# paninski-lab/lightning-pose

Hardware: AMD Instinct MI355X
Metric: training frames/sec (whole node), ResNet-50 384x384 17-kp semi-sup (higher is better)
Workload: dtype bf16; 1 GPU; C2/C3: ResNet-50 SemiSupervisedHeatmapTracker 384x384, K=17, 64 labeled + 128 unlabeled frames per GPU, heatmap_mse + temporal + pca_singleview + unimodal_mse, Adam (backbone lr=0 as at step 0), bf16-mixed; global_batch=192, parallelism=dp1, sync_batchnorm=False, decode_prune=plain kernels (chosen from the maps)

## Files before the change

include/lp_hip.h:

```cpp
#ifndef LP_HIP_H
#define LP_HIP_H

#include <stddef.h>
#include <stdint.h>

#ifdef __cplusplus
extern "C" {
#endif

typedef void* lp_stream_t;

int lp_config_reload_env(void);

enum {
    LP_OK = 0,
    LP_ERR_ARGUMENT = -1,
    LP_ERR_UNSUPPORTED = -2,
};

enum { LP_TF_NONE = 0, LP_TF_SINGLE = 1, LP_TF_PER_FRAME = 2, LP_TF_PER_VIEW = 3 };

#define LP_HIP_ABI_VERSION 142
int lp_version(void);
const char* lp_strerror(int code);


typedef struct lp_decode_tables {
    const int* row_base;
    const float* row_taps;
    const int* col_start;
    const float* col_taps;
    const int* colT_start;
    const float* colT_taps;
    int ty, tx, tc;
} lp_decode_tables;

typedef struct lp_frame_map {
    const float* transforms;
    int tf_mode;
    const float* bbox;
    int bbox_stride;
    int kp_per_view;
    float model_h, model_w;
} lp_frame_map;

// ... 49 lines not shown

int lp_temporal_fwd_bwd(const float* kp, const float* conf, int S, int K, const float* eps_per_kp, float prob_threshold,
                        float* loss, float* grad_unit, lp_stream_t stream);

int lp_pca_fwd_bwd(const float* kp, int S, int K, const int* index, int rows, int points, const float* mean,
                   const float* kept_eigenvectors, int ncomp, float epsilon, float* loss, float* grad_unit, lp_stream_t stream);

int lp_rmse_fwd(const float* kp_targ, const float* kp_pred, int n_points, float* loss, lp_stream_t stream);
int lp_loss_combine(const float* const* x, const float* w, const float* a, int n, float* weighted, float* total, lp_stream_t stream);
int lp_loss_combine_bwd(const float* w, const float* a, int n, const float* g_weighted, const float* g_total, float* gx, lp_stream_t stream);

typedef struct lp_conv_geom {
    int B, Hi, Wi, Ci;
    int Ho, Wo, Co;
    int R, S, stride, pad;
} lp_conv_geom;

#define LP_CONV_KERNEL_IGEMM 0
#define LP_CONV_KERNEL_PIPE 1
#define LP_CONV_KERNEL_WGRAD 2
#define LP_CONV_KERNEL_WGRAD_PIPE 3
#define LP_CONV_KERNEL_PIPE_HALO 4
#define LP_CONV_KERNEL_STEM_WGRAD_NB 8
#define LP_CONV_KERNEL_RES2D 5
int lp_conv_last_kernel(void);

int lp_conv_fwd(const void* x, const void* w, const lp_conv_geom* geom, const float* bias, void* out_bf16, float* out_f32, int ldo,
                int n_store, lp_stream_t stream);
int lp_conv_dgrad(const void* dy, const void* wd, const lp_conv_geom* geom, const float* bias, const void* addend,
                  const void* relu_mask, void* dx_bf16, float* dx_f32, int ldo, int n_store, int skip_empty_classes,
                  lp_stream_t stream);
typedef struct lp_gemm_batch {
    int nb, nh;
    long long a_b, a_h, b_b, b_h, c_b, c_h;
} lp_gemm_batch;
int lp_gemm_nt(const void* a, int lda, const void* b, int ldb, void* c_bf16, float* c_f32, int ldc, int M, int N, int K, int n_store,
               const float* bias, const lp_gemm_batch* batch, lp_stream_t stream);
int lp_gemm_tn(const void* x, int ldx, const void* y, int ldy, void* out_bf16, int ldo, int M, int J, int N, const lp_gemm_batch* batch,
               lp_stream_t stream);
int lp_attn_fwd(const void* qkv_bf16, int ld_qkv, int k_off, int v_off, int B, int nh, int T, float scale, void* p_bf16, int ldp,
                void* out_bf16, int ldo, lp_stream_t stream);
int lp_attn_bwd_kv(const void* qkv_bf16, int ld_qkv, int v_off, const void* d_out_bf16, int ld_do, const void* p_bf16, int ldp, const float* d_rows,
                   int B, int nh, int T, float scale, void* ds_bf16, void* dqkv_bf16, int ld_dqkv, int dk_off, int dv_off, lp_stream_t stream);
int lp_attn_rowdot(const void* a_bf16, const void* b_bf16, int rows, int nh, int ld, float* out, lp_stream_t stream);
int lp_attn_dscores(const void* d_out, int ld_do, const void* v, int ldv, const void* p_bf16, const float* d_rows, int d_row_stride,
                    long long d_b, long long d_h, float scale, void* ds_bf16, int ldc, int M, int N, int K, const lp_gemm_batch* batch,
// ... 174 lines not shown
```

lightning-pose_amd/_lib.py:

```python

from __future__ import annotations

import ctypes as C
import os

_HERE = os.path.dirname(os.path.abspath(__file__))
LIB_PATH = os.environ.get("LP_HIP_LIB") or os.path.join(_HERE, "liblp_hip.so")


class LpHipUnavailable(RuntimeError):
    """liblp_hip.so could not be loaded, or an op was given a non-ROCm tensor.  There is no fallback path."""


class LpHipError(RuntimeError):
    pass


class DecodeTables(C.Structure):
    _fields_ = [("row_base", C.c_void_p), ("row_taps", C.c_void_p), ("col_start", C.c_void_p),
                ("col_taps", C.c_void_p), ("colT_start", C.c_void_p), ("colT_taps", C.c_void_p),
                ("ty", C.c_int), ("tx", C.c_int), ("tc", C.c_int)]


class FrameMap(C.Structure):
# ... 6 lines not shown


class BnFuse(C.Structure):
    _fields_ = [("z", C.c_void_p), ("mean", C.c_void_p), ("invstd", C.c_void_p), ("gamma", C.c_void_p), ("beta", C.c_void_p),
                ("mask_from_z", C.c_int), ("relu_bits", C.c_void_p), ("sums", C.c_void_p), ("seg_images", C.c_int), ("addend_half", C.c_int)]


class FrameNorm(C.Structure):
    _fields_ = [("mean", C.c_float * 3), ("std", C.c_float * 3)]


class FrameAugment(C.Structure):
    _fields_ = [("has_matrix", C.c_int), ("matrix", C.c_float * 6), ("brightness", C.c_float), ("contrast", C.c_float),
                ("contrast_center", C.c_float), ("shot_factor", C.c_float), ("seed", C.c_ulonglong)]


class GemmBatch(C.Structure):
    _fields_ = [("nb", C.c_int), ("nh", C.c_int)] + [(n, C.c_longlong) for n in ("a_b", "a_h", "b_b", "b_h", "c_b", "c_h")]


HM_MSE, HM_KL, HM_JS = 0, 1, 2
CONV_KERNEL_IGEMM, CONV_KERNEL_PIPE, CONV_KERNEL_WGRAD, CONV_KERNEL_WGRAD_PIPE, CONV_KERNEL_PIPE_HALO, CONV_KERNEL_RES2D = 0, 1, 2, 3, 4, 5
CONV_KERNEL_STEM_WGRAD_NB = 8
BORDER_RENORM, BORDER_CLAMP = 0, 1
TF_NONE, TF_SINGLE, TF_PER_FRAME, TF_PER_VIEW = 0, 1, 2, 3

ABI_VERSION = 142

_P, _I, _F, _L, _Z = C.c_void_p, C.c_int, C.c_float, C.c_long, C.c_size_t

PROTOTYPES = {
    "lp_version": (_I, []),
    "lp_strerror": (C.c_char_p, [_I]),
    "lp_config_reload_env": (_I, []),
    "lp_decode_window": (_I, [_I, _I]),
    "lp_decode_fwd": (_I, [_P, _I, _I, _I, _I, _I, _F, C.POINTER(DecodeTables), C.POINTER(FrameMap), _P, _P, _P, _P, _I, _P]),
    "lp_decode_bwd": (_I, [_P, _I, _I, _I, _I, _I, _F, C.POINTER(DecodeTables), C.POINTER(FrameMap), _P, _P, _P, _P, _I, _I, _P]),
    "lp_frame_map_apply": (_I, [_P, _I, _I, C.POINTER(FrameMap), _I, _P, _P]),
    "lp_heatmap_gen": (_I, [_P, _P, _I, _I, _I, _I, _I, _I, _F, _P, _P]),
    "lp_heatmap_gen_bwd": (_I, [_P, _P, _I, _I, _I, _I, _I, _I, _F, _P, _P, _P]),
    "lp_temporal_heatmap_workspace_bytes": (_Z, [_I, _I]),
    "lp_temporal_heatmap_fwd": (_I, [_I, _P, _P, _I, _I, _I, _I, _P, _F, _P, _P, _P]),
    "lp_temporal_heatmap_bwd": (_I, [_I, _P, _I, _I, _I, _I, _P, _P, _P, _I, _P]),
    "lp_heatmap_confidence": (_I, [_P, _P, _I, _I, _I, _I, _I, _P, _P]),
    "lp_heatmap_mse_workspace_bytes": (_Z, [_I, _I]),
    "lp_heatmap_mse_fwd": (_I, [_P, _P, _I, _I, _I, _I, _P, _P, _P]),
    "lp_heatmap_mse_bwd": (_I, [_P, _P, _I, _I, _I, _I, _P, _P, _P, _I, _P]),
    "lp_heatmap_loss_fwd": (_I, [_I, _P, _P, _I, _I, _I, _I, _P, _P, _P]),
    "lp_heatmap_loss_bwd": (_I, [_I, _P, _P, _I, _I, _I, _I, _P, _P, _P, _I, _P]),
    "lp_unimodal_mse_fwd": (_I, [_P, _P, _P, _I, _I, _I, _I, _I, _I, _F, _F, _P, _P, _P]),
# ... 138 lines not shown
```

lightning-pose_amd/csrc/api.hip:

```cpp
#include "lp_common.h"

#include <stdlib.h>

#include <atomic>

extern "C" int lp_version(void) { return LP_HIP_ABI_VERSION; }

namespace lp {
static int env_int(const char* name, int dflt) {
    const char* e = getenv(name);
    return (e == nullptr || *e == 0) ? dflt : atoi(e);
}
static LpSwitches read_switches() {
    LpSwitches s;
    s.conv_pipe = env_int("LP_CONV_PIPE", 1);
    s.conv_halo = env_int("LP_CONV_HALO", 1);
    s.conv_res2d = env_int("LP_CONV_RES2D", 1);
    s.infer_pipe = env_int("LP_INFER_PIPE", 1);
    s.gemm_pipe = env_int("LP_GEMM_PIPE", 1);
    s.wgrad_pipe = env_int("LP_WGRAD_PIPE", 1);
    s.stem_2d = env_int("LP_STEM_2D", 1);
    s.stem_wgrad_nb = env_int("LP_STEM_WGRAD_NB", 1);
    s.pool_v2 = env_int("LP_POOL_V2", 1);
    s.bn_bwd_wgs_per_cu = env_int("LP_BN_BWD_WGS_PER_CU", 5);
    if (s.bn_bwd_wgs_per_cu < 1 || s.bn_bwd_wgs_per_cu > 5) s.bn_bwd_wgs_per_cu = 5;
    s.conv_max_wgs = env_int("LP_CONV_MAX_WGS", 0);
    return s;
}
static std::atomic<const LpSwitches*> g_switches{new LpSwitches(read_switches())};
const LpSwitches& lp_switches() { return *g_switches.load(std::memory_order_acquire); }
}

extern "C" int lp_config_reload_env(void) {
    lp::g_switches.store(new lp::LpSwitches(lp::read_switches()), std::memory_order_release);
    return LP_OK;
}

extern "C" const char* lp_strerror(int code) {
    if (code == LP_OK) return "ok";
    if (code == LP_ERR_ARGUMENT) return "invalid argument (null pointer or non-positive dimension)";
    if (code == LP_ERR_UNSUPPORTED) return "shape not covered by the instantiated kernels";
    if (code > 0) return hipGetErrorString((hipError_t)code);
    return "unknown lp_hip error";
// ... 2 lines not shown
```

lightning-pose_amd/csrc/conv.hip:

```cpp
#include <stdlib.h>

#include "lp_common.h"

namespace lp {

constexpr int kBM = 128;
constexpr int kBK = 64;
constexpr int kLD = kBK + 8;

struct ConvGeom {
    int B, Hi, Wi, Ci;
    int Ho, Wo, Co;
    int R, S, stride, pad;
};

struct ConvEpilogue {
    unsigned short* out_bf16;
    float* out_f32;
    int ldo;
    int n_store;
    const float* bias;
    const unsigned short* addend;
    const unsigned short* relu_mask;
    const unsigned char* relu_bits;
// ... 509 lines not shown
            if (kt + 1 < KT) load_step(kt + 1);
            mma_kstep<NT>(sA[cur], sB[cur], wm, wn, lane, acc);
            if (kt + 1 < KT) store_step(cur ^ 1);
            __syncthreads();
        }
        vt += gridDim.x;
        const unsigned zd = zdn;
        if (vt >= ntiles) {
            epilogue(m0, n0, zo, zd);
            if (ep.stats_sums != nullptr) stats_flush();
            break;
        }
        setup(vt);
        load_step(0, MODE != kModeDgrad);
        epilogue(m0, n0, zo, zd);
        if (MODE == kModeDgrad) load_b_deferred();
        __syncthreads();
    }
}

}

#include "conv_pipe.h"
#include "conv_res2d.h"

namespace lp {

struct TnExt {
    unsigned short* out;
    int ldx, ldy, ldo;
    int nh;
    unsigned x_zb, x_zh;
    unsigned y_zb, y_zh;
    unsigned o_zb, o_zh;
    float* col_sums;
};

#ifndef LP_WGRAD_DEEP
#define LP_WGRAD_DEEP 1
#endif
constexpr bool kWgradDeep = LP_WGRAD_DEEP != 0;

template <int BN, bool STEM, bool CS = false>
__global__ __launch_bounds__(256) void conv_wgrad_kernel(const unsigned short* __restrict__ X, const unsigned short* __restrict__ DY,
                                                         unsigned x_bytes, unsigned dy_bytes, ConvGeom g, int M, int Kw, int tiles,
                                                         int tiles_n, int m_per_split, FastDiv div_hw, FastDiv div_wo,
// ... 574 lines not shown
    const void *pa = x, *qb = dy;
    unsigned pa_bytes = x_bytes, qb_bytes = dy_bytes;
    if (p.swap) {
        wg = WgradPipeGeom{g.B, g.Ho, g.Wo, g.Ho, g.Wo, g.Co, 1, 1, 1, 0, p.Ka, p.Cb, 1};
        pa = dy, qb = x, pa_bytes = dy_bytes, qb_bytes = x_bytes;
    } else {
        const int plain = g.R == 1 && g.S == 1 && g.stride == 1 && g.pad == 0 && g.Hi == g.Ho && g.Wi == g.Wo;
        wg = WgradPipeGeom{g.B, g.Hi, g.Wi, g.Ho, g.Wo, g.Ci, g.R, g.S, g.stride, g.pad, p.Ka, p.Cb, plain};
    }
    const int tiles = p.tiles_a * p.tiles_b;
    const FastDiv dhw = make_fastdiv(g.Ho * g.Wo), dwo = make_fastdiv(g.Wo);
    g_last_conv_kernel = LP_CONV_KERNEL_WGRAD_PIPE;
    const int sa = p.swap ? Kw : 1, sb = p.swap ? 1 : Kw;
    if (p.bn == 128) {
        hipLaunchKernelGGL((conv_wgrad_pipe_kernel<128>), dim3(tiles * p.split), dim3(512), 0, st, (const unsigned short*)pa,
                           (const unsigned short*)qb, pa_bytes, qb_bytes, wg, M, tiles, p.tiles_b, p.per, dhw, dwo, ws);
        hipLaunchKernelGGL((wgrad_pipe_reduce_kernel<128>), dim3(tiles * 256 * 128 / 64), dim3(256), 0, st, ws, p.split, tiles, p.tiles_b, p.Ka,
                           p.Cb, sa, sb, dw);
    } else {
        hipLaunchKernelGGL((conv_wgrad_pipe_kernel<64>), dim3(tiles * p.split), dim3(512), 0, st, (const unsigned short*)pa,
                           (const unsigned short*)qb, pa_bytes, qb_bytes, wg, M, tiles, p.tiles_b, p.per, dhw, dwo, ws);
        hipLaunchKernelGGL((wgrad_pipe_reduce_kernel<64>), dim3(tiles * 256 * 64 / 64), dim3(256), 0, st, ws, p.split, tiles, p.tiles_b, p.Ka,
                           p.Cb, sa, sb, dw);
    }
}

static bool geom_ok(const lp_conv_geom* c) {
    return c && c->B > 0 && c->Hi > 0 && c->Wi > 0 && c->Ci > 0 && c->Ho > 0 && c->Wo > 0 && c->Co > 0 && c->R > 0 && c->S > 0 &&
           c->stride > 0 && c->pad >= 0;
}

static ConvGeom to_geom(const lp_conv_geom* c) {
    ConvGeom g{c->B, c->Hi, c->Wi, c->Ci, c->Ho, c->Wo, c->Co, c->R, c->S, c->stride, c->pad};
    return g;
}

}

static int conv_fwd_impl(const void* x, const void* w, const lp_conv_geom* geom, const float* bias, void* out_bf16, float* out_f32, int ldo,
                         int n_store, const lp_bn_fuse* bn, lp_stream_t stream) {
    using namespace lp;
    LP_REQUIRE(x && w && geom_ok(geom) && (out_bf16 || out_f32) && ldo > 0);
    ConvGeom g = to_geom(geom);
    if (g.Ci % kBK != 0 || g.R * g.S > 32 || (long long)g.B * g.Hi * g.Wi * g.Ci >= (1LL << 31) ||
        (long long)g.B * g.Ho * g.Wo * ldo >= (1LL << 32))
        return LP_ERR_UNSUPPORTED;
// ... 277 lines not shown
    if (split > ksteps) split = ksteps;
    if (split < 1) split = 1;
    p.per = ((ksteps + split - 1) / split) * lp::kBK;
    p.split = (M + p.per - 1) / p.per;
    p.tj = 2, p.tn = 1, p.wide = false;
    p.ws_floats = (size_t)p.split * 2 * 4 * 2 * 16 * 64;
    return p;
}

extern "C" size_t lp_conv_wgrad_workspace_bytes(const lp_conv_geom* geom, int split_hint) {
    using namespace lp;
    if (!geom_ok(geom)) return 0;
    ConvGeom g = to_geom(geom);
    const bool stem = (g.Ci == 4 && g.R == 7);
    const int Kw = stem ? 256 : g.R * g.S * g.Ci;
    size_t fl = plan_wgrad(g.B * g.Ho * g.Wo, Kw, g.Co, split_hint, kWgradWgs).ws_floats;
    if (stem && stem_wgrad_nb_ok(g)) {
        const size_t nb = plan_stem_wgrad_nb(g.B * g.Ho * g.Wo, split_hint).ws_floats;
        if (nb > fl) fl = nb;
    }
    if (!stem) {
        const WgradPipePlan pp = plan_wgrad_pipe(g, split_hint, true);
        if (pp.ok && pp.ws_floats > fl) fl = pp.ws_floats;
    }
    return fl * sizeof(float);
}

static int conv_wgrad_impl(const void* x, const void* dy, const lp_conv_geom* geom, float* dw, float* dbias, int split_hint, void* workspace,
                           size_t workspace_bytes, lp_stream_t stream) {
    using namespace lp;
    LP_REQUIRE(x && dy && geom_ok(geom) && dw && workspace);
    ConvGeom g = to_geom(geom);
    if (g.Ci % 8 != 0 || g.Co % 8 != 0 || (long long)g.B * g.Hi * g.Wi * g.Ci >= (1LL << 31) ||
        (long long)g.B * g.Ho * g.Wo * g.Co >= (1LL << 31))
        return LP_ERR_UNSUPPORTED;
    const int M = g.B * g.Ho * g.Wo, Kw = g.R * g.S * g.Ci;
    const unsigned x_bytes = (unsigned)(2ull * g.B * g.Hi * g.Wi * g.Ci), dy_bytes = (unsigned)(2ull * M * g.Co);
    const WgradPlan p = plan_wgrad(M, Kw, g.Co, split_hint, kWgradWgs);
    LP_REQUIRE(workspace_bytes >= p.ws_floats * sizeof(float));
    hipStream_t st = (hipStream_t)stream;
    float* ws = (float*)workspace;
    const int wpe = lp_switches().wgrad_pipe;
    if (!dbias && conv_pipe_enabled() && wpe != 0) {
        const WgradPipePlan pp = plan_wgrad_pipe(g, split_hint, wpe == 2);
        if (pp.ok && workspace_bytes >= pp.ws_floats * sizeof(float)) {
            launch_wgrad_pipe(pp, x, dy, g, dw, ws, st);
            return launch_status();
        }
    }
    g_last_conv_kernel = LP_CONV_KERNEL_WGRAD;
    const int tiles = p.tj * p.tn;
    TnExt ext{};
    ext.col_sums = dbias;
    const dim3 grid(tiles * p.split), block(256);
    const FastDiv dhw = make_fastdiv(g.Ho * g.Wo), dwo = make_fastdiv(g.Wo);
    const unsigned short *xs = (const unsigned short*)x, *dys = (const unsigned short*)dy;
#define LP_WGRAD_LAUNCH(BN_, CS_)                                                                                                \
    hipLaunchKernelGGL((conv_wgrad_kernel<BN_, false, CS_>), grid, block, 0, st, xs, dys, x_bytes, dy_bytes, g, M, Kw, tiles, p.tn, \
                       p.per, dhw, dwo, ws, ext)
    if (p.wide) {
        if (dbias) LP_WGRAD_LAUNCH(128, true);
        else LP_WGRAD_LAUNCH(128, false);
        launch_wgrad_reduce<128>(ws, p.split, tiles, p.tn, Kw, g.Co, dw, st);
    } else {
        if (dbias) LP_WGRAD_LAUNCH(64, true);
// ... 117 lines not shown
```

lightning-pose_amd/csrc/conv_pipe.h:

```cpp
#pragma once

#include <type_traits>

namespace lp {

#ifndef LP_HALO_KEY_ROW
#define LP_HALO_KEY_ROW 0
#endif
#ifndef LP_HALO_STAGES
#define LP_HALO_STAGES 3
#endif
#ifndef LP_FWD_CORNER_PAD
#define LP_FWD_CORNER_PAD 0
#endif
#ifndef LP_PIPE_SPREAD
#define LP_PIPE_SPREAD 1
#endif
constexpr bool kSpread = LP_PIPE_SPREAD != 0;
constexpr int kPM = 256;
constexpr int kPRowB = 128;

#if defined(__HIP_DEVICE_COMPILE__)
#define LP_WAIT_VM(n) asm volatile("s_waitcnt vmcnt(" #n ")" ::: "memory")
#define LP_RAW_BARRIER()                   \
    do {                                   \
        asm volatile("" ::: "memory");     \
        __builtin_amdgcn_s_barrier();      \
        asm volatile("" ::: "memory");     \
    } while (0)
#define LP_WAIT_LGKM_TOUCH3(n, a, b, c) asm volatile("s_waitcnt lgkmcnt(" #n ")" : "+v"(a), "+v"(b), "+v"(c)::"memory")
#define LP_WAIT_LGKM_TOUCH4(n, a, b, c, d) asm volatile("s_waitcnt lgkmcnt(" #n ")" : "+v"(a), "+v"(b), "+v"(c), "+v"(d)::"memory")
#else
#define LP_WAIT_VM(n) ((void)0)
#define LP_RAW_BARRIER() __syncthreads()
#define LP_WAIT_LGKM_TOUCH3(n, a, b, c) ((void)0)
#define LP_WAIT_LGKM_TOUCH4(n, a, b, c, d) ((void)0)
#endif

__device__ __forceinline__ void store8(unsigned short* p, u16x8 v) { *reinterpret_cast<u16x8*>(p) = v; }
// ... 669 lines not shown
    const int bchunk = (BN == 128) ? ((lane & 15) ^ ((brow & 3) << 2)) : ((lane & 7) ^ (((brow >> 1) & 1) << 2));
    const unsigned boff = (unsigned)(b0 + bchunk * 8) * 2u;
    const int hw = g.Ho * g.Wo;

    unsigned is_a[4], is_b[NLB];
    unsigned char* is_dst = smem;
    const bool same = !g.plain && g.stride == 1 && g.Hi == g.Ho && g.Wi == g.Wo && hw >= kBK;
    const int qb64 = kBK / hw, qh64 = (kBK - qb64 * hw) / g.Wo, qw64 = kBK - qb64 * hw - qh64 * g.Wo;
    const int lo_h = max(0, g.pad - tr), span_h = min(g.Ho, g.Hi + g.pad - tr) - lo_h;
    const int lo_w = max(0, g.pad - ts), span_w = min(g.Wo, g.Wi + g.pad - ts) - lo_w;
    const unsigned tap_off = (unsigned)(((tr - g.pad) * g.Wi + (ts - g.pad)) * g.Ca + tcn) * 2u;
    int rho[4], rwo[4];
    if (same) {
#pragma unroll
        for (int p = 0; p < 4; ++p) {
            const int m = m_begin + p * 16 + arow;
            const int mm = m < M ? m : 0;
            const int rem = mm - fdiv(mm, div_hw) * hw;
            rho[p] = fdiv(rem, div_wo);
            rwo[p] = rem - rho[p] * g.Wo;
        }
    }
    auto prep_step = [&](int st, int kt) {
        const int mk = m_begin + kt * kBK;
#pragma unroll
        for (int p = 0; p < 4; ++p) {
            const int m = mk + p * 16 + arow;
            unsigned off;
            bool ok = ja_ok && m < m_end && kt < KT;
            if (g.plain) {
                off = (unsigned)(m * g.Ca + tcn) * 2u;
            } else if (same) {
                ok = ok && (unsigned)(rho[p] - lo_h) < (unsigned)span_h && (unsigned)(rwo[p] - lo_w) < (unsigned)span_w;
                off = (unsigned)m * (unsigned)(g.Ca * 2) + tap_off;
                rwo[p] += qw64;
                const int c = rwo[p] >= g.Wo ? 1 : 0;
                rwo[p] -= c ? g.Wo : 0;
                rho[p] += qh64 + c;
                rho[p] -= rho[p] >= g.Ho ? g.Ho : 0;
            } else {
                const int mm = ok ? m : 0;
                const int b = fdiv(mm, div_hw), rem = mm - b * hw;
                const int ho = fdiv(rem, div_wo), wo = rem - ho * g.Wo;
                const int hi = ho * g.stride - g.pad + tr, wi = wo * g.stride - g.pad + ts;
                ok = ok && hi >= 0 && hi < g.Hi && wi >= 0 && wi < g.Wi;
                off = (unsigned)(((b * g.Hi + hi) * g.Wi + wi) * g.Ca + tcn) * 2u;
            }
// ... 27 lines not shown
        const int e0 = wn * (NT * 32) + nt * 32 + fcol;
        fob[nt] = (unsigned)(kStageA + frow * kRowB + (((e0 >> 3) ^ swb) << 4) + (e0 & 7) * 2);
    }
    f32x16 acc[2][NT];
#pragma unroll
    for (int mt = 0; mt < 2; ++mt)
#pragma unroll
        for (int nt = 0; nt < NT; ++nt)
#pragma unroll
            for (int e = 0; e < 16; ++e) acc[mt][nt][e] = 0.f;

    auto mma_stage = [&](int st) {
        const unsigned char* sb = smem + st * kStage;
        bf16x8 a[2][2], b[2][NT];
        const unsigned char* pa[2];
        const unsigned char* pb[NT];
#pragma unroll
        for (int mt = 0; mt < 2; ++mt) pa[mt] = sb + foa[mt];
#pragma unroll
        for (int nt = 0; nt < NT; ++nt) pb[nt] = sb + fob[nt];
        auto fetch = [&](auto kk_c, int set) {
            constexpr int kk = decltype(kk_c)::value;
            typedef __attribute__((ext_vector_type(8))) short s16x8_t;
#pragma unroll
            for (int mt = 0; mt < 2; ++mt) {
                const s16x4_t lo = lds_read_tr16_async_off<kk * 16 * kRowA>(pa[mt]), hi = lds_read_tr16_async_off<kk * 16 * kRowA + 4 * kRowA>(pa[mt]);
                const s16x8_t v = {lo[0], lo[1], lo[2], lo[3], hi[0], hi[1], hi[2], hi[3]};
                a[set][mt] = __builtin_bit_cast(bf16x8, v);
            }
#pragma unroll
            for (int nt = 0; nt < NT; ++nt) {
                const s16x4_t lo = lds_read_tr16_async_off<kk * 16 * kRowB>(pb[nt]), hi = lds_read_tr16_async_off<kk * 16 * kRowB + 4 * kRowB>(pb[nt]);
                const s16x8_t v = {lo[0], lo[1], lo[2], lo[3], hi[0], hi[1], hi[2], hi[3]};
                b[set][nt] = __builtin_bit_cast(bf16x8, v);
            }
        };
        auto ready = [&](int set, bool last) {
            if (NT == 2) {
                if (last) LP_WAIT_LGKM_TOUCH4(0, a[set][0], a[set][1], b[set][0], b[set][NT - 1]);
                else LP_WAIT_LGKM_TOUCH4(8, a[set][0], a[set][1], b[set][0], b[set][NT - 1]);
            } else {
                if (last) LP_WAIT_LGKM_TOUCH3(0, a[set][0], a[set][1], b[set][0]);
                else LP_WAIT_LGKM_TOUCH3(6, a[set][0], a[set][1], b[set][0]);
            }
        };
        auto slice = [&](auto kk_c) {
            constexpr int kk = decltype(kk_c)::value;
            if constexpr (kk + 1 < kBK / 16) fetch(std::integral_constant<int, kk + 1>{}, (kk + 1) & 1);
            __builtin_amdgcn_sched_barrier(0);
            ready(kk & 1, kk + 1 == kBK / 16);
#pragma unroll
            for (int mt = 0; mt < 2; ++mt)
#pragma unroll
                for (int nt = 0; nt < NT; ++nt)
                    acc[mt][nt] = __builtin_amdgcn_mfma_f32_32x32x16_bf16(a[kk & 1][mt], b[kk & 1][nt], acc[mt][nt], 0, 0, 0);
            constexpr int NL = 4 + NLB;
            if (kk == 0) {
                issue_load(0);
                issue_load(1);
            } else if (kk == 1) {
                issue_load(2);
                if (NL == 6) issue_load(3);
            } else if (kk == 2) {
                issue_load(NL == 6 ? 4 : 3);
            } else {
                issue_load(NL - 1);
            }
            __builtin_amdgcn_sched_barrier(0);
        };
        fetch(std::integral_constant<int, 0>{}, 0);
        slice(std::integral_constant<int, 0>{});
        slice(std::integral_constant<int, 1>{});
        slice(std::integral_constant<int, 2>{});
        slice(std::integral_constant<int, 3>{});
    };

    prep_step(0, 0);
#pragma unroll
// ... 61 lines not shown
```

lightning-pose_amd/csrc/lp_common.h:

```cpp
#pragma once

#include <hip/hip_runtime.h>
#include <stdint.h>

#include "../../include/lp_hip.h"

namespace lp {

constexpr int kWave = 64;

typedef __attribute__((ext_vector_type(8))) __bf16 bf16x8;
typedef __attribute__((ext_vector_type(8))) unsigned short u16x8;
typedef __attribute__((ext_vector_type(4))) unsigned short u16x4;
typedef __attribute__((ext_vector_type(4))) float f32x4;
typedef __attribute__((ext_vector_type(16))) float f32x16;

__device__ __forceinline__ float bf16_to_f32(unsigned short b) { return __uint_as_float(((unsigned)b) << 16); }

#if defined(__HIP_DEVICE_COMPILE__)
typedef __attribute__((ext_vector_type(2))) __bf16 bf16x2_t;
typedef __attribute__((ext_vector_type(2))) float f32x2_t;
__device__ __forceinline__ unsigned short f32_to_bf16(float f) { return __builtin_bit_cast(unsigned short, (__bf16)f); }
__device__ __forceinline__ unsigned pack_bf16x2(float lo, float hi) {
    const f32x2_t v = {lo, hi};
// ... 224 lines not shown

constexpr long long kFxPoison = 5LL << 60;
constexpr long long kFxPoisonSeen = 1LL << 59;
__device__ __forceinline__ void fx_add(lp_fxsum* p, float t) {
    double td = (double)t;
    if (!(fabs(td) <= 0x1p127 * 2.0)) {
        atomicMax(&p->lo, kFxPoison);
        return;
    }
    td = fmin(fmax(td, -0x1p49), 0x1p49);
    const double h = rint(td * 0x1p12);
    const long long hi = (long long)h;
    const long long lo = (long long)rint((td - h * 0x1p-12) * 0x1p60);
    atomicAdd(reinterpret_cast<unsigned long long*>(&p->hi), (unsigned long long)hi);
    atomicAdd(reinterpret_cast<unsigned long long*>(&p->lo), (unsigned long long)lo);
}
__device__ __forceinline__ float fx_value(const lp_fxsum* p) {
    const long long lo = p->lo;
    if (lo >= kFxPoisonSeen || lo <= -kFxPoisonSeen) return __int_as_float(0x7fc00000);
    return (float)((double)p->hi * 0x1p-12 + (double)lo * 0x1p-60);
}

struct LpSwitches {
    int conv_pipe, conv_halo, conv_res2d, infer_pipe, gemm_pipe, wgrad_pipe, stem_2d, stem_wgrad_nb, pool_v2, conv_max_wgs, bn_bwd_wgs_per_cu;
};
const LpSwitches& lp_switches();

inline int launch_status() {
    hipError_t e = hipGetLastError();
    return e == hipSuccess ? LP_OK : (int)e;
}

}

#define LP_REQUIRE(cond)                    \
    do {                                    \
        if (!(cond)) return LP_ERR_ARGUMENT; \
    } while (0)
```

lightning-pose_amd/engine.py:

```python

from __future__ import annotations

import ctypes as C
import math
import os
from dataclasses import dataclass, field

import torch
import torch.distributed as dist

from . import _lib
from ._lib import check
from . import ops
from .ops import _p

BN_EPS = 1e-5
BN_MOMENTUM = 0.1
CPAD = 64


@dataclass
class ConvP:
    name: str
    kind: str
# ... 194 lines not shown
            return t
        return torch.zeros(n, device=self.device, dtype=torch.float32)

    def _zeros_fx(self, n: int) -> torch.Tensor:
        return self._zeros_f32(4 * n).view(torch.int64)

    def _timed(self, tag: str, flops: float, fn, nbytes: float = 0.0, layer: str = ""):
        if self.profile is None:
            return fn()
        e0, e1 = torch.cuda.Event(enable_timing=True), torch.cuda.Event(enable_timing=True)
        e0.record()
        out = fn()
        e1.record()
        if tag.startswith("conv_") and hasattr(self._lib, "lp_conv_last_kernel"):
            k = self._lib.lp_conv_last_kernel()
            if k == _lib.CONV_KERNEL_PIPE:
                tag = tag.replace("conv_igemm_kernel", "conv_pipe_kernel")
            elif k == _lib.CONV_KERNEL_PIPE_HALO:
                tag = tag.replace("conv_igemm_kernel", "conv_pipe_kernel").replace(">", ",halo>")
            elif k == _lib.CONV_KERNEL_RES2D:
                tag = tag.replace("conv_igemm_kernel<64,", "conv_res2d_kernel<").replace("conv_igemm_kernel<64>", "conv_res2d_kernel<fwd>")
            elif k == _lib.CONV_KERNEL_WGRAD_PIPE:
                tag = tag.replace("conv_wgrad_kernel", "conv_wgrad_pipe_kernel")
        self.profile.append((tag, flops, e0, e1, nbytes, layer))
        return out

    def _wgrad(self, x, dy, g, dw: torch.Tensor, stem: bool = False, dbias: torch.Tensor | None = None) -> None:
        need = self._lib.lp_conv_wgrad_workspace_bytes(C.byref(g), 0)
        if self._wgrad_ws is None or self._wgrad_ws.numel() < need:
            self._join_side_stream()
            self._wgrad_ws = torch.empty(max(need, 96 << 20), device=self.device, dtype=torch.uint8)
        fn = self._lib.lp_stem_wgrad if stem else self._lib.lp_conv_wgrad
        what = "lp_stem_wgrad" if stem else "lp_conv_wgrad"
        if dbias is not None:
            what = "lp_conv_wgrad_bias"
            fn = lambda x_, dy_, g_, dw_, split, ws, nws, st: self._lib.lp_conv_wgrad_bias(x_, dy_, g_, dw_, _p(dbias), split, ws, nws, st)
        if (self.device.type != "cuda" or not self.wgrad_side_stream or self.profile is not None
                or os.environ.get("LP_WGRAD_SIDE_STREAM", "1") == "0"):
            check(fn(_p(x), _p(dy), C.byref(g), _p(dw), 0, _p(self._wgrad_ws), self._wgrad_ws.numel(), ops._stream()), what)
            return
        if self._side is None:
            self._side = torch.cuda.Stream(device=self.device)
        main = torch.cuda.current_stream(self.device)
        self._side.wait_stream(main)
        self._side_keep.append((x, dy))
        with torch.cuda.stream(self._side):
# ... 702 lines not shown
```

Before: 4679 frames/s.

## Add tap-reuse wgrad kernel for 3x3 stride-1 convolutions

Adds a new weight-gradient kernel for 3x3 stride-1 pad-1 convs. It loads one contiguous window of input rows per k-step into LDS and computes all nine taps from shifted views of it, masking border taps with ballot-derived kill masks. This replaces a per-tap im2col-style gather, so each input element is fetched once instead of up to nine times. A split-K planner with a cost model picks the split count, and a separate reduce kernel sums the partials into dW. The path is enabled by default when the pipe wgrad is active; it also adds compile-time probe macros (off by default) to the existing pipe kernel.

```diff
diff --git a/include/lp_hip.h b/include/lp_hip.h
--- a/include/lp_hip.h
+++ b/include/lp_hip.h
@@ -20,7 +20,7 @@
 
 enum { LP_TF_NONE = 0, LP_TF_SINGLE = 1, LP_TF_PER_FRAME = 2, LP_TF_PER_VIEW = 3 };
 
-#define LP_HIP_ABI_VERSION 142
+#define LP_HIP_ABI_VERSION 143
 int lp_version(void);
 const char* lp_strerror(int code);
 
@@ -116,6 +116,7 @@
 #define LP_CONV_KERNEL_WGRAD_PIPE 3
 #define LP_CONV_KERNEL_PIPE_HALO 4
 #define LP_CONV_KERNEL_STEM_WGRAD_NB 8
+#define LP_CONV_KERNEL_WGRAD_TAPS 9
 #define LP_CONV_KERNEL_RES2D 5
 int lp_conv_last_kernel(void);
 
diff --git a/lightning-pose_amd/_lib.py b/lightning-pose_amd/_lib.py
--- a/lightning-pose_amd/_lib.py
+++ b/lightning-pose_amd/_lib.py
@@ -52,10 +52,11 @@
 HM_MSE, HM_KL, HM_JS = 0, 1, 2
 CONV_KERNEL_IGEMM, CONV_KERNEL_PIPE, CONV_KERNEL_WGRAD, CONV_KERNEL_WGRAD_PIPE, CONV_KERNEL_PIPE_HALO, CONV_KERNEL_RES2D = 0, 1, 2, 3, 4, 5
 CONV_KERNEL_STEM_WGRAD_NB = 8
+CONV_KERNEL_WGRAD_TAPS = 9
 BORDER_RENORM, BORDER_CLAMP = 0, 1
 TF_NONE, TF_SINGLE, TF_PER_FRAME, TF_PER_VIEW = 0, 1, 2, 3
 
-ABI_VERSION = 142
+ABI_VERSION = 143
 
 _P, _I, _F, _L, _Z = C.c_void_p, C.c_int, C.c_float, C.c_long, C.c_size_t
 
diff --git a/lightning-pose_amd/csrc/api.hip b/lightning-pose_amd/csrc/api.hip
--- a/lightning-pose_amd/csrc/api.hip
+++ b/lightning-pose_amd/csrc/api.hip
@@ -19,6 +19,7 @@
     s.infer_pipe = env_int("LP_INFER_PIPE", 1);
     s.gemm_pipe = env_int("LP_GEMM_PIPE", 1);
     s.wgrad_pipe = env_int("LP_WGRAD_PIPE", 1);
+    s.wgrad_taps = env_int("LP_WGRAD_TAPS", 1);
     s.stem_2d = env_int("LP_STEM_2D", 1);
     s.stem_wgrad_nb = env_int("LP_STEM_WGRAD_NB", 1);
     s.pool_v2 = env_int("LP_POOL_V2", 1);
diff --git a/lightning-pose_amd/csrc/conv.hip b/lightning-pose_amd/csrc/conv.hip
--- a/lightning-pose_amd/csrc/conv.hip
+++ b/lightning-pose_amd/csrc/conv.hip
@@ -555,6 +555,7 @@
 }
 
 #include "conv_pipe.h"
+#include "conv_wgrad_taps.h"
 #include "conv_res2d.h"
 
 namespace lp {
@@ -1175,6 +1176,71 @@
                            (const unsigned short*)qb, pa_bytes, qb_bytes, wg, M, tiles, p.tiles_b, p.per, dhw, dwo, ws);
         hipLaunchKernelGGL((wgrad_pipe_reduce_kernel<64>), dim3(tiles * 256 * 64 / 64), dim3(256), 0, st, ws, p.split, tiles, p.tiles_b, p.Ka,
                            p.Cb, sa, sb, dw);
+    }
+}
+
+struct WgradTapsPlan {
+    bool ok;
+    int bn, tiles_ci, tiles_co, rows, na, split, per;
+    bool refetch;
+    size_t ws_floats;
+};
+
+static WgradTapsPlan plan_wgrad_taps(const ConvGeom& g, int split_hint, bool force = false) {
+    WgradTapsPlan p{};
+    if (g.R != 3 || g.S != 3 || g.stride != 1 || g.pad != 1 || g.Hi != g.Ho || g.Wi != g.Wo || g.Ci % 64 != 0 || g.Co % 64 != 0) return p;
+    p.rows = kBK + 2 * g.Wo + 2;
+    p.bn = (g.Co % 128 == 0 && p.rows <= kTapsRowsMax128) ? 128 : 64;
+    if (p.rows > (p.bn == 128 ? kTapsRowsMax128 : kTapsRowsMax64)) return p;
+    p.na = (p.rows + 63) / 64;
+    p.refetch = true;
+    p.tiles_ci = g.Ci / 64;
+    p.tiles_co = g.Co / p.bn;
+    const int M = g.B * g.Ho * g.Wo, tiles = p.tiles_ci * p.tiles_co;
+    const int cus = pipe_max_wgs();
+    const int ksteps = (M + kBK - 1) / kBK;
+    int split = split_hint;
+    if (split <= 0) {
+        const double mfma_clk = 2304.0 * p.bn / 128.0, fill_clk = (p.rows * 128.0 + kBK * p.bn * 2.0) / 50.0;
+        const double stepc = fill_clk > mfma_clk ? fill_clk / mfma_clk : 1.0;
+        double best = 1e30;
+        for (int s = 1; s <= 2 * cus && s <= ksteps; ++s) {
+            if (s != 1 && (tiles * s) % cus > 0 && (tiles * (s + 1) + cus - 1) / cus == (tiles * s + cus - 1) / cus) continue;
+            const double rounds = (double)((tiles * s + cus - 1) / cus), per = (double)((ksteps + s - 1) / s);
+            const double cost = rounds * per * stepc + 0.04 * (p.bn / 128.0) * s * tiles + 2.0 * rounds * stepc;
+            if (cost < best) best = cost, split = s;
+        }
+        if (split <= 0) split = 1;
+    }
+    if (split > ksteps) split = ksteps;
+    if (split < 1) split = 1;
+    p.per = ((ksteps + split - 1) / split) * kBK;
+    p.split = (M + p.per - 1) / p.per;
+    p.ws_floats = (size_t)p.split * tiles * 8 * 9 * 16 * 64;
+    if (!force && split_hint <= 0) {
+        const double partial_us = 2.0 * 4.0 * 9 * 64 * p.bn * (double)p.split * tiles / 4e6;
+        const double mfma_us = (p.per / kBK) * 2304.0 * (p.bn / 128.0) / 2400.0;
+        if (partial_us > mfma_us) return p;
+    }
+    p.ok = true;
+    return p;
+}
+
+static void launch_wgrad_taps(const WgradTapsPlan& p, const void* x, const void* dy, const ConvGeom& g, float* dw, float* ws, hipStream_t st) {
+    const int M = g.B * g.Ho * g.Wo;
+    const unsigned x_bytes = (unsigned)(2ull * M * g.Ci), dy_bytes = (unsigned)(2ull * M * g.Co);
+    const WgradTapsGeom tg{g.Ho, g.Wo, g.Ci, g.Co, M, p.rows, p.na};
+    const int tiles = p.tiles_ci * p.tiles_co;
+    const FastDiv dhw = make_fastdiv(g.Ho * g.Wo), dwo = make_fastdiv(g.Wo);
+    g_last_conv_kernel = LP_CONV_KERNEL_WGRAD_TAPS;
+    if (p.bn == 128) {
+        hipLaunchKernelGGL((conv_wgrad_taps_kernel<128>), dim3(tiles * p.split), dim3(512), 0, st, (const unsigned short*)x,
+                           (const unsigned short*)dy, x_bytes, dy_bytes, tg, M, tiles, p.tiles_co, p.per, dhw, dwo, ws);
+        hipLaunchKernelGGL((wgrad_taps_reduce_kernel<128>), dim3(tiles * 8 * 9 * 16), dim3(256), 0, st, ws, p.split, tiles, p.tiles_co, g.Ci, dw);
+    } else {
+        hipLaunchKernelGGL((conv_wgrad_taps_kernel<64>), dim3(tiles * p.split), dim3(512), 0, st, (const unsigned short*)x,
+                           (const unsigned short*)dy, x_bytes, dy_bytes, tg, M, tiles, p.tiles_co, p.per, dhw, dwo, ws);
+        hipLaunchKernelGGL((wgrad_taps_reduce_kernel<64>), dim3(tiles * 4 * 9 * 16), dim3(256), 0, st, ws, p.split, tiles, p.tiles_co, g.Ci, dw);
     }
 }
 
@@ -1498,6 +1564,8 @@
     if (!stem) {
         const WgradPipePlan pp = plan_wgrad_pipe(g, split_hint, true);
         if (pp.ok && pp.ws_floats > fl) fl = pp.ws_floats;
+        const WgradTapsPlan tp = plan_wgrad_taps(g, split_hint, true);
+        if (tp.ok && tp.ws_floats > fl) fl = tp.ws_floats;
     }
     return fl * sizeof(float);
 }
@@ -1517,6 +1585,13 @@
     hipStream_t st = (hipStream_t)stream;
     float* ws = (float*)workspace;
     const int wpe = lp_switches().wgrad_pipe;
+    if (!dbias && conv_pipe_enabled() && lp_switches().wgrad_taps != 0 && wpe == 1) {
+        const WgradTapsPlan tp = plan_wgrad_taps(g, split_hint, lp_switches().wgrad_taps == 2);
+        if (tp.ok && workspace_bytes >= tp.ws_floats * sizeof(float)) {
+            launch_wgrad_taps(tp, x, dy, g, dw, ws, st);
+            return launch_status();
+        }
+    }
     if (!dbias && conv_pipe_enabled() && wpe != 0) {
         const WgradPipePlan pp = plan_wgrad_pipe(g, split_hint, wpe == 2);
         if (pp.ok && workspace_bytes >= pp.ws_floats * sizeof(float)) {
diff --git a/lightning-pose_amd/csrc/conv_pipe.h b/lightning-pose_amd/csrc/conv_pipe.h
--- a/lightning-pose_amd/csrc/conv_pipe.h
+++ b/lightning-pose_amd/csrc/conv_pipe.h
@@ -15,6 +15,9 @@
 #endif
 #ifndef LP_PIPE_SPREAD
 #define LP_PIPE_SPREAD 1
+#endif
+#ifndef LP_WGRAD_PROBE
+#define LP_WGRAD_PROBE 0
 #endif
 constexpr bool kSpread = LP_PIPE_SPREAD != 0;
 constexpr int kPM = 256;
@@ -730,7 +733,7 @@
         }
     }
     auto prep_step = [&](int st, int kt) {
-        const int mk = m_begin + kt * kBK;
+        const int mk = m_begin + ((LP_WGRAD_PROBE == 3 && kt >= 2 && kt < KT) ? 0 : kt) * kBK;
 #pragma unroll
         for (int p = 0; p < 4; ++p) {
             const int m = mk + p * 16 + arow;
@@ -804,6 +807,17 @@
         auto fetch = [&](auto kk_c, int set) {
             constexpr int kk = decltype(kk_c)::value;
             typedef __attribute__((ext_vector_type(8))) short s16x8_t;
+#if LP_WGRAD_PROBE == 2
+            int c = kk + lane;
+            LP_OPAQUE(c);
+            const s16x8_t cv = {(short)c, (short)c, (short)c, (short)c, (short)c, (short)c, (short)c, (short)c};
+#pragma unroll
+            for (int mt = 0; mt < 2; ++mt) a[set][mt] = __builtin_bit_cast(bf16x8, cv);
+#pragma unroll
+            for (int nt = 0; nt < NT; ++nt) b[set][nt] = __builtin_bit_cast(bf16x8, cv);
+            (void)pa, (void)pb;
+            return;
+#endif
 #pragma unroll
             for (int mt = 0; mt < 2; ++mt) {
                 const s16x4_t lo = lds_read_tr16_async_off<kk * 16 * kRowA>(pa[mt]), hi = lds_read_tr16_async_off<kk * 16 * kRowA + 4 * kRowA>(pa[mt]);
@@ -835,7 +849,7 @@
             for (int mt = 0; mt < 2; ++mt)
 #pragma unroll
                 for (int nt = 0; nt < NT; ++nt)
-                    acc[mt][nt] = __builtin_amdgcn_mfma_f32_32x32x16_bf16(a[kk & 1][mt], b[kk & 1][nt], acc[mt][nt], 0, 0, 0);
+                    if (LP_WGRAD_PROBE != 1) acc[mt][nt] = __builtin_amdgcn_mfma_f32_32x32x16_bf16(a[kk & 1][mt], b[kk & 1][nt], acc[mt][nt], 0, 0, 0);
             constexpr int NL = 4 + NLB;
             if (kk == 0) {
                 issue_load(0);
diff --git a/lightning-pose_amd/csrc/conv_wgrad_taps.h b/lightning-pose_amd/csrc/conv_wgrad_taps.h
--- /dev/null
+++ b/lightning-pose_amd/csrc/conv_wgrad_taps.h
@@ -0,0 +1,249 @@
+#pragma once
+
+#include <utility>
+
+namespace lp {
+
+#ifndef LP_TAPS_DEPTH
+#define LP_TAPS_DEPTH 3
+#endif
+
+constexpr int kTapsStage = 48 * 1024;
+constexpr int kTapsRowsMax128 = 256, kTapsRowsMax64 = 320;
+
+struct WgradTapsGeom {
+    int Ho, Wo, Ci, Co;
+    int Mtot;
+    int rows;
+    int na;
+};
+
+template <class F, int... I>
+__device__ __forceinline__ void taps_unroll(F&& f, std::integer_sequence<int, I...>) {
+    (f(std::integral_constant<int, I>{}), ...);
+}
+
+template <int N>
+__device__ __forceinline__ void taps_wait_lgkm(s16x4_t& a, s16x4_t& b, s16x4_t& c, s16x4_t& d) {
+#if defined(__HIP_DEVICE_COMPILE__)
+    asm volatile("s_waitcnt lgkmcnt(%4)" : "+v"(a), "+v"(b), "+v"(c), "+v"(d) : "n"(N) : "memory");
+#endif
+}
+
+typedef __attribute__((ext_vector_type(4))) unsigned taps_u32x4;
+
+__device__ __forceinline__ taps_u32x4 taps_kill(unsigned bits) {
+    taps_u32x4 k;
+#pragma unroll
+    for (int j = 0; j < 4; ++j) k[j] = (((bits >> (2 * j)) & 1u) ? 0xffffu : 0u) | (((bits >> (2 * j + 1)) & 1u) ? 0xffff0000u : 0u);
+    return k;
+}
+
+template <int BN>
+__global__ __launch_bounds__(512) void conv_wgrad_taps_kernel(const unsigned short* __restrict__ X, const unsigned short* __restrict__ DY,
+                                                              unsigned x_bytes, unsigned dy_bytes, WgradTapsGeom g, int M, int tiles,
+                                                              int tiles_co, int m_per_split, FastDiv div_hw, FastDiv div_wo,
+                                                              float* __restrict__ ws) {
+    constexpr int KG = 128 / BN;
+    constexpr int NSL = 4 / KG;
+    constexpr int Q = NSL * 9;
+    constexpr int D = LP_TAPS_DEPTH;
+    constexpr int NLB = BN / 64;
+    constexpr int NAMAX = BN == 128 ? kTapsRowsMax128 / 64 : kTapsRowsMax64 / 64;
+    constexpr int kRowX = 128, kRowB = BN * 2;
+    constexpr int kStageX = NAMAX * 64 * kRowX;
+    static_assert(kStageX + kBK * kRowB == kTapsStage, "stage layout");
+    static_assert(D >= 2 && D <= 4, "fragment ring depth");
+    __shared__ __attribute__((aligned(16))) unsigned char smem[3 * kTapsStage];
+
+    const int tid = threadIdx.x, lane = tid & 63;
+    const int wave = __builtin_amdgcn_readfirstlane(tid >> 6);
+    const int cih = wave & 1, cobw = (wave >> 1) & (BN / 32 - 1), kg = BN == 128 ? 0 : wave >> 2;
+    const int work = xcd_remap(blockIdx.x, gridDim.x);
+    const int slice = work / tiles, tile = work - slice * tiles;
+    const int ci0 = (tile / tiles_co) * 64, co0 = (tile % tiles_co) * BN;
+    const int m_begin = slice * m_per_split, m_end = min(M, m_begin + m_per_split);
+    const int KT = (m_end - m_begin + kBK - 1) / kBK;
+    const buf_rsrc rsrc_x = make_buf_rsrc(X, x_bytes), rsrc_b = make_buf_rsrc(DY, dy_bytes);
+    const int na = g.na;
+
+    int xp0[NAMAX];
+    unsigned xcoff[NAMAX];
+#pragma unroll
+    for (int i = 0; i < NAMAX; ++i) {
+        const int j = i * 64 + wave * 8 + (lane >> 3);
+        const int chunk = (lane & 7) ^ (((j >> 1) & 1) << 2);
+        xp0[i] = j < g.rows ? m_begin - g.Wo - 1 + j : -(1 << 30);
+        xcoff[i] = (unsigned)(ci0 + chunk * 8) * 2u;
+    }
+    const int brow = (BN == 128) ? wave * 4 + (lane >> 4) : wave * 8 + (lane >> 3);
+    const int bchunk = (BN == 128) ? ((lane & 15) ^ ((brow & 3) << 2)) : ((lane & 7) ^ (((brow >> 1) & 1) << 2));
+    const unsigned boff = (unsigned)(co0 + bchunk * 8) * 2u;
+
+    unsigned is_x[NAMAX], is_b[NLB];
+    unsigned char* is_dst = smem;
+    auto prep_step = [&](int st, int kt) {
+        const bool live = kt < KT;
+#pragma unroll
+        for (int i = 0; i < NAMAX; ++i) {
+            const int p = xp0[i] + kt * kBK;
+            const bool ok = live && p >= 0 && p < g.Mtot;
+            is_x[i] = ok ? (unsigned)p * (unsigned)(g.Ci * 2) + xcoff[i] : ~0u;
+        }
+#pragma unroll
+        for (int q = 0; q < NLB; ++q) {
+            const int m = m_begin + kt * kBK + q * 32 + brow;
+            is_b[q] = (live && m < m_end) ? (unsigned)m * (unsigned)(g.Co * 2) + boff : ~0u;
+        }
+        is_dst = smem + st * kTapsStage;
+    };
+    auto issue_load = [&](int i) {
+        if (i < NAMAX) {
+            if (i < na) buf_load16_lds(rsrc_x, is_dst + (i * 64 + wave * 8) * kRowX, is_x[i < NAMAX ? i : 0], 0u);
+        } else if (BN == 128) {
+            buf_load16_lds(rsrc_b, is_dst + kStageX + ((i - NAMAX) * 32 + wave * 4) * kRowB, is_b[(i - NAMAX) % NLB], 0u);
+        } else {
+            buf_load16_lds(rsrc_b, is_dst + kStageX + (wave * 8) * kRowB, is_b[0], 0u);
+        }
+    };
+
+    const int fq = lane >> 4, fi = lane & 15;
+    const int frow = (fq >> 1) * 8 + (fi >> 2), fcol = (fq & 1) * 16 + (fi & 3) * 4;
+    unsigned foa[9], fob;
+    {
+        const int e0 = cih * 32 + fcol;
+#pragma unroll
+        for (int t = 0; t < 9; ++t) {
+            const int jr = (t / 3) * g.Wo + (t % 3) + kg * (NSL * 16) + frow;
+            foa[t] = (unsigned)(jr * kRowX + (((e0 >> 3) ^ (((jr >> 1) & 1) << 2)) << 4) + (e0 & 7) * 2);
+        }
+        const int eb = cobw * 32 + fcol, rb = kg * (NSL * 16) + frow;
+        const int swb = (BN == 128) ? ((rb & 3) << 2) : (((rb >> 1) & 1) << 2);
+        fob = (unsigned)(kStageX + rb * kRowB + (((eb >> 3) ^ swb) << 4) + (eb & 7) * 2);
+    }
+    const int sh8 = (lane >> 5) * 8;
+
+    f32x16 acc[9];
+#pragma unroll
+    for (int t = 0; t < 9; ++t)
+#pragma unroll
+        for (int e = 0; e < 16; ++e) acc[t][e] = 0.f;
+
+    typedef __attribute__((ext_vector_type(8))) short s16x8_t;
+    auto mma_stage = [&](int st, int kt) {
+        const unsigned char* sb = smem + st * kTapsStage;
+        unsigned long long k_c0, k_c2, k_r0, k_r2;
+        {
+            const int m = m_begin + kt * kBK + lane;
+            const int rem = m - fdiv(m, div_hw) * div_hw.d;
+            const int ho = fdiv(rem, div_wo), wo = rem - ho * g.Wo;
+            k_c0 = __ballot(wo == 0);
+            k_c2 = __ballot(wo == g.Wo - 1);
+            k_r0 = __ballot(ho == 0);
+            k_r2 = __ballot(ho == g.Ho - 1);
+        }
+        s16x4_t alo[D], ahi[D], blo[2], bhi[2];
+        taps_u32x4 bm[3], kr0 = {0u, 0u, 0u, 0u}, kr2 = {0u, 0u, 0u, 0u};
+        bool rows_hit = false;
+        auto issue = [&](auto qc) {
+            constexpr int q = decltype(qc)::value, kk = q / 9, t = q % 9;
+            if constexpr (t == 0) {
+                blo[kk & 1] = lds_read_tr16_async_off<kk * 16 * kRowB>(sb + fob);
+                bhi[kk & 1] = lds_read_tr16_async_off<kk * 16 * kRowB + 4 * kRowB>(sb + fob);
+            }
+            alo[q % D] = lds_read_tr16_async_off<kk * 16 * kRowX>(sb + foa[t]);
+            ahi[q % D] = lds_read_tr16_async_off<kk * 16 * kRowX + 4 * kRowX>(sb + foa[t]);
+        };
+        auto step = [&](auto qc) {
+            constexpr int q = decltype(qc)::value, kk = q / 9, t = q % 9, r = t / 3, s = t % 3;
+            constexpr int last = (q + D - 1 < Q - 1) ? q + D - 1 : Q - 1;
+            constexpr int pending = 2 * (last - q) + 2 * ((last / 9) - (q / 9));
+            taps_wait_lgkm<pending>(alo[q % D], ahi[q % D], blo[kk & 1], bhi[kk & 1]);
+            const s16x8_t av = {alo[q % D][0], alo[q % D][1], alo[q % D][2], alo[q % D][3], ahi[q % D][0], ahi[q % D][1], ahi[q % D][2], ahi[q % D][3]};
+            taps_u32x4 a = __builtin_bit_cast(taps_u32x4, av);
+            if constexpr (q + D < Q) issue(std::integral_constant<int, q + D>{});
+            if constexpr (t == 0) {
+                const s16x8_t bv = {blo[kk & 1][0], blo[kk & 1][1], blo[kk & 1][2], blo[kk & 1][3], bhi[kk & 1][0], bhi[kk & 1][1], bhi[kk & 1][2], bhi[kk & 1][3]};
+                const int sh = (kg * NSL + kk) * 16;
+                bm[1] = __builtin_bit_cast(taps_u32x4, bv);
+                bm[0] = bm[1], bm[2] = bm[1];
+                if ((unsigned)(k_c0 >> sh) & 0xffffu) bm[0] &= ~taps_kill((unsigned)(k_c0 >> sh) >> sh8);
+                if ((unsigned)(k_c2 >> sh) & 0xffffu) bm[2] &= ~taps_kill((unsigned)(k_c2 >> sh) >> sh8);
+                rows_hit = ((unsigned)((k_r0 | k_r2) >> sh) & 0xffffu) != 0u;
+                if (rows_hit) {
+                    kr0 = taps_kill((unsigned)(k_r0 >> sh) >> sh8);
+                    kr2 = taps_kill((unsigned)(k_r2 >> sh) >> sh8);
+                }
+            }
+            if constexpr (r != 1) {
+                if (rows_hit) a &= ~(r == 0 ? kr0 : kr2);
+            }
+            acc[t] = __builtin_amdgcn_mfma_f32_32x32x16_bf16(__builtin_bit_cast(bf16x8, a), __builtin_bit_cast(bf16x8, bm[s]), acc[t], 0, 0, 0);
+            constexpr int P0 = BN == 128 ? 3 : 2, PS = BN == 128 ? 5 : 2;
+            if constexpr (q >= P0 && (q - P0) % PS == 0 && (q - P0) / PS < NAMAX + NLB) issue_load((q - P0) / PS);
+        };
+        taps_unroll([&](auto qc) { issue(qc); }, std::make_integer_sequence<int, D>{});
+        taps_unroll(step, std::make_integer_sequence<int, Q>{});
+    };
+
+    prep_step(0, 0);
+#pragma unroll
+    for (int i = 0; i < NAMAX + NLB; ++i) issue_load(i);
+    prep_step(1, 1);
+#pragma unroll
+    for (int i = 0; i < NAMAX + NLB; ++i) issue_load(i);
+    int cur = 0;
+    for (int kt = 0; kt < KT; ++kt) {
+        switch (na + NLB) {
+            case 2: LP_WAIT_VM(2); break;
+            case 3: LP_WAIT_VM(3); break;
+            case 4: LP_WAIT_VM(4); break;
+            case 5: LP_WAIT_VM(5); break;
+            case 6: LP_WAIT_VM(6); break;
+            default: LP_WAIT_VM(7); break;
+        }
+        LP_RAW_BARRIER();
+        prep_step(cur == 0 ? 2 : cur - 1, kt + 2);
+        mma_stage(cur, kt);
+        cur = cur == 2 ? 0 : cur + 1;
+    }
+    LP_WAIT_VM(0);
+    float* dst = ws + ((((size_t)slice * tiles + tile) * 8 + wave) * (9 * 16)) * 64 + lane;
+#pragma unroll
+    for (int t = 0; t < 9; ++t)
+#pragma unroll
+        for (int e = 0; e < 16; ++e) dst[(t * 16 + e) * 64] = acc[t][e];
+}
+
+template <int BN>
+__global__ __launch_bounds__(256) void wgrad_taps_reduce_kernel(const float* __restrict__ ws, int slices, int tiles, int tiles_co, int Ci,
+                                                                float* __restrict__ dW) {
+    constexpr int KG = 128 / BN;
+    constexpr int PER_WAVE = 9 * 16 * 64, PER_TILE = 8 * PER_WAVE;
+    __shared__ float part[4][64];
+    const int lane = threadIdx.x & 63, w = threadIdx.x >> 6;
+    int t = blockIdx.x;
+    const int e = t & 15;
+    t >>= 4;
+    const int tap = t % 9;
+    t /= 9;
+    const int wv = t % (8 / KG), tile = t / (8 / KG);
+    const size_t total = (size_t)tiles * PER_TILE;
+    const size_t i = (size_t)tile * PER_TILE + (size_t)wv * PER_WAVE + (size_t)(tap * 16 + e) * 64 + lane;
+    float s0 = 0.f;
+    for (int sl = w; sl < slices; sl += 4) {
+        s0 += ws[(size_t)sl * total + i];
+        if (KG == 2) s0 += ws[(size_t)sl * total + i + 4 * PER_WAVE];
+    }
+    part[w][lane] = s0;
+    __syncthreads();
+    if (w == 0) {
+        const float sum = (part[0][lane] + part[1][lane]) + (part[2][lane] + part[3][lane]);
+        const int cih = wv & 1, cobw = wv >> 1;
+        const int ci = (tile / tiles_co) * 64 + cih * 32 + (e & 3) + 8 * (e >> 2) + 4 * (lane >> 5);
+        const int co = (tile % tiles_co) * BN + cobw * 32 + (lane & 31);
+        dW[((size_t)co * 9 + tap) * Ci + ci] += sum;
+    }
+}
+
+}
diff --git a/lightning-pose_amd/csrc/lp_common.h b/lightning-pose_amd/csrc/lp_common.h
--- a/lightning-pose_amd/csrc/lp_common.h
+++ b/lightning-pose_amd/csrc/lp_common.h
@@ -270,7 +270,7 @@
 }
 
 struct LpSwitches {
-    int conv_pipe, conv_halo, conv_res2d, infer_pipe, gemm_pipe, wgrad_pipe, stem_2d, stem_wgrad_nb, pool_v2, conv_max_wgs, bn_bwd_wgs_per_cu;
+    int conv_pipe, conv_halo, conv_res2d, infer_pipe, gemm_pipe, wgrad_pipe, wgrad_taps, stem_2d, stem_wgrad_nb, pool_v2, conv_max_wgs, bn_bwd_wgs_per_cu;
 };
 const LpSwitches& lp_switches();
 
diff --git a/lightning-pose_amd/engine.py b/lightning-pose_amd/engine.py
--- a/lightning-pose_amd/engine.py
+++ b/lightning-pose_amd/engine.py
@@ -240,6 +240,8 @@
                 tag = tag.replace("conv_igemm_kernel<64,", "conv_res2d_kernel<").replace("conv_igemm_kernel<64>", "conv_res2d_kernel<fwd>")
             elif k == _lib.CONV_KERNEL_WGRAD_PIPE:
                 tag = tag.replace("conv_wgrad_kernel", "conv_wgrad_pipe_kernel")
+            elif k == _lib.CONV_KERNEL_WGRAD_TAPS:
+                tag = tag.replace("conv_wgrad_kernel", "conv_wgrad_taps_kernel")
         self.profile.append((tag, flops, e0, e1, nbytes, layer))
         return out
 
```

Result: no change. 4684 frames/s, median of 3 (+0.1%).
